# darcamo/pyphysim

Hardware: AMD Instinct MI355X
Metric: Monte Carlo realizations/sec (whole node) + SER abs-error vs ref (higher is better)
Workload: dtype f64

## Files before the change

pyphysim_amd/csrc/bm_f64.hpp:

```cpp
#pragma once
#include <cstdint>

#ifndef MCLE_BM_TABLE
#define MCLE_BM_TABLE static __device__ const
#endif
#ifndef MCLE_BM_FN
#define MCLE_BM_FN __device__ __forceinline__
#endif
#ifndef MCLE_BM_RSQ
#define MCLE_BM_RSQ(a) __builtin_amdgcn_rsq(a)
#endif
#ifndef MCLE_BM_FMA
#define MCLE_BM_FMA(a, b, c) __builtin_fma(a, b, c)
#endif
#ifndef MCLE_BM_RINT
#define MCLE_BM_RINT(a) __builtin_rint(a)
#endif

#ifndef MCLE_BM_ALIGNBIT
#ifdef __HIPCC__
#define MCLE_BM_ALIGNBIT(hi, lo, s) __builtin_amdgcn_alignbit(hi, lo, s)
#else
#define MCLE_BM_ALIGNBIT(hi, lo, s) ((uint32_t)(((((uint64_t)(hi)) << 32) | (uint64_t)(uint32_t)(lo)) >> (s)))
#endif
// ... 115 lines not shown
        st = t[1];
    } else {
        ct = reinterpret_cast<const double*>(entry)[0];
        st = reinterpret_cast<const double*>(entry)[1];
    }
    const double r = ang - *reinterpret_cast<const double*>(reinterpret_cast<const char*>(ttheta) + (off >> 1));
    const double s2 = r * r;
    double p = MCLE_BM_FMA(s2, -1.0 / 5040.0, 1.0 / 120.0);
    p = MCLE_BM_FMA(s2, p, -1.0 / 6.0);
    const double sr = MCLE_BM_FMA(r * s2, p, r);
    double q = MCLE_BM_FMA(s2, -1.0 / 720.0, 1.0 / 24.0);
    q = MCLE_BM_FMA(s2, q, -0.5);
    const double cm = s2 * q;
    c = ct + MCLE_BM_FMA(-st, sr, ct * cm);
    s = st + MCLE_BM_FMA(ct, sr, st * cm);
}

struct BmFetched {
    int d, e;
    uint32_t x1;
    BmPair lg;
    BmPair cs;
    double theta;
};

MCLE_BM_FN BmFetched bm_sample_fetch(uint32_t x0, uint32_t x1, const double* tlogq, const double* ttheta, const double* ttrig) {
    BmFetched t;
    const double ud = (double)x0 + 0.5;
    const uint64_t bits = __builtin_bit_cast(uint64_t, ud);
    const uint32_t hi = (uint32_t)(bits >> 32);
    const uint32_t f = MCLE_BM_ALIGNBIT(hi, (uint32_t)bits, 20);
    t.d = MCLE_BM_SBFE((int)f, 0, 26);
    t.e = (int)(hi + 0x82000u - ((1023u + 32u) << 20)) >> 20;
    const uint32_t offl = (((f >> 1) + (1u << 24)) >> 21) & 0x7F0u;
    t.lg = *reinterpret_cast<const BmPair*>(reinterpret_cast<const char*>(tlogq) + offl);
    t.x1 = x1;
    const uint32_t offt = ((x1 >> 21) + 8u) & 0xFF0u;
    t.cs = *reinterpret_cast<const BmPair*>(reinterpret_cast<const char*>(ttrig) + offt);
    t.theta = *reinterpret_cast<const double*>(reinterpret_cast<const char*>(ttheta) + (offt >> 1));
    return t;
}

MCLE_BM_FN void bm_sample_finish(const BmFetched& t, double sigma, double& re, double& im) {
    const double inv_cq = t.lg[0], lnc = t.lg[1];
    const double r = (double)t.d * inv_cq;
    const double r2 = r * r;
    const double a0 = MCLE_BM_FMA(r, 1.0 / 3.0, -0.5);
    const double a1 = MCLE_BM_FMA(r, 0.2, -0.25);
    const double a2 = MCLE_BM_FMA(r, 1.0 / 7.0, -1.0 / 6.0);
    const double q = MCLE_BM_FMA(r2, MCLE_BM_FMA(r2, a2, a1), a0);
    const double small = MCLE_BM_FMA(r2, q, r);
    const double big = MCLE_BM_FMA((double)t.e, 0x1.62e42fefa39efp-1, lnc);
    const double rad = sigma * bm_sqrt(-(big + small));
    const double ang = (double)t.x1 * 0x1.921fb54442d18p-30;
    const double ct = t.cs[0], st = t.cs[1];
    const double rr = ang - t.theta;
    const double s2 = rr * rr;
    double p = MCLE_BM_FMA(s2, -1.0 / 5040.0, 1.0 / 120.0);
    p = MCLE_BM_FMA(s2, p, -1.0 / 6.0);
    const double sr = MCLE_BM_FMA(rr * s2, p, rr);
    double qq = MCLE_BM_FMA(s2, -1.0 / 720.0, 1.0 / 24.0);
    qq = MCLE_BM_FMA(s2, qq, -0.5);
    const double cm = s2 * qq;
    const double c = ct + MCLE_BM_FMA(-st, sr, ct * cm);
    const double s = st + MCLE_BM_FMA(ct, sr, st * cm);
    re = rad * c;
    im = rad * s;
}

MCLE_BM_FN void bm_sincos_packed(uint32_t x1, double& c, double& s, const double* tpk) {
    const double ang = (double)x1 * 0x1.921fb54442d18p-30;
    const uint32_t k = ((x1 >> 24) + 1u) >> 1;
    const double ct = tpk[4 * k], st = tpk[4 * k + 1];
    const double r = ang - tpk[4 * k + 2];
    const double s2 = r * r;
    double p = MCLE_BM_FMA(s2, -1.0 / 5040.0, 1.0 / 120.0);
    p = MCLE_BM_FMA(s2, p, -1.0 / 6.0);
    const double sr = MCLE_BM_FMA(r * s2, p, r);
    double q = MCLE_BM_FMA(s2, -1.0 / 720.0, 1.0 / 24.0);
    q = MCLE_BM_FMA(s2, q, -0.5);
    const double cm = s2 * q;
    c = ct + MCLE_BM_FMA(-st, sr, ct * cm);
    s = st + MCLE_BM_FMA(ct, sr, st * cm);
}
#ifdef __HIPCC__
constexpr int kBmPackedDoubles = 129 * 4;
__device__ __forceinline__ void bm_trig_packed_to_lds(double* s_pk, int tid, int nthreads) {
    for (int i = tid; i < kBmThetaLen; i += nthreads) {
        s_pk[4 * i] = kBmTrig[2 * i];
        s_pk[4 * i + 1] = kBmTrig[2 * i + 1];
        s_pk[4 * i + 2] = kBmTheta[i];
        s_pk[4 * i + 3] = 0.0;
    }
}
#endif

MCLE_BM_FN void bm_sincos_rad(double x, double& c, double& s) {
    const double C1 = 0x1.45f306dc9c883p-3;
    const double C2 = -0x1.6b01ec5417056p-57;
    const double p = x * C1;
    const double e = MCLE_BM_FMA(x, C1, -p) + x * C2;
    const double kd = MCLE_BM_RINT(p * 4.0);
    const int k = (int)kd;
    const double rt = MCLE_BM_FMA(kd, -0.25, p) + e;
    const double r = rt * 0x1.921fb54442d18p+2;
    const double z = r * r;
// ... 24 lines not shown
```

pyphysim_amd/csrc/philox.hpp:

```cpp
#pragma once
#include "common.hpp"
#include "bm_f64.hpp"

namespace mcle {

enum : uint32_t { STREAM_DATA = 0, STREAM_NOISE = 1, STREAM_CHAN = 2, STREAM_PHASE = 3, STREAM_PILOT = 4 };

struct Words4 {
    uint32_t w[4];
};

__host__ __device__ __forceinline__ Words4 philox4x32_10(uint32_t c0, uint32_t c1, uint32_t c2,
                                                         uint32_t c3, uint32_t k0, uint32_t k1) {
#pragma unroll
    for (int r = 0; r < 10; ++r) {
        const uint64_t p0 = (uint64_t)0xD2511F53u * c0;
        const uint64_t p1 = (uint64_t)0xCD9E8D57u * c2;
#if defined(__HIP_DEVICE_COMPILE__)
        const uint32_t n0 = __builtin_amdgcn_bitop3_b32((uint32_t)(p1 >> 32), c1, k0, 0x96);
        const uint32_t n2 = __builtin_amdgcn_bitop3_b32((uint32_t)(p0 >> 32), c3, k1, 0x96);
#else
        const uint32_t n0 = (uint32_t)(p1 >> 32) ^ c1 ^ k0;
        const uint32_t n2 = (uint32_t)(p0 >> 32) ^ c3 ^ k1;
#endif
// ... 19 lines not shown
          r1((uint32_t)(realization >> 32)) {}
    __host__ __device__ __forceinline__ Words4 block(uint32_t stream, uint32_t blk) const {
        return philox4x32_10(blk, stream, r0, r1, k0, k1);
    }
};

__device__ __forceinline__ float2 cn_from_words(uint32_t x0, uint32_t x1, float sigma) {
    const float u = fmaf((float)x0, 0x1p-32f, 0x1p-33f);
    const float v = (float)x1 * 0x1p-32f;
    const float rad = __builtin_amdgcn_sqrtf((-0.69314718055994531f * sigma * sigma) * __builtin_amdgcn_logf(u));
    float2 z;
    z.x = rad * __builtin_amdgcn_cosf(v);
    z.y = rad * __builtin_amdgcn_sinf(v);
    return z;
}
__device__ __forceinline__ double2 cn_from_words(uint32_t x0, uint32_t x1, double sigma) {
    const double rad = sigma * bm_sqrt(bm_neg_log_q(x0));
    double s, c;
    bm_sincos(x1, c, s);
    double2 z;
    z.x = rad * c;
    z.y = rad * s;
    return z;
}

__device__ __forceinline__ double2 cn_from_words_lds(uint32_t x0, uint32_t x1, double sigma, const double* s_bm) {
    const double rad = sigma * bm_sqrt(bm_neg_log_q(x0, s_bm));
    double s, c;
    bm_sincos(x1, c, s, s_bm + kBmLogLen, s_bm + kBmLogLen + kBmThetaLen);
    double2 z;
    z.x = rad * c;
    z.y = rad * s;
    return z;
}

__device__ __forceinline__ double2 cn_from_words_lds_pairs(uint32_t x0, uint32_t x1, double sigma, const double* s_bm) {
    const double rad = sigma * bm_sqrt(bm_neg_log_q<true>(x0, s_bm));
    double s, c;
    bm_sincos<true>(x1, c, s, s_bm + kBmLogLen + kBmTrigLen, s_bm + kBmLogLen);
    double2 z;
    z.x = rad * c;
    z.y = rad * s;
    return z;
}

__device__ __forceinline__ BmFetched cn_fetch_lds_pairs(uint32_t x0, uint32_t x1, const double* s_bm) {
    return bm_sample_fetch(x0, x1, s_bm, s_bm + kBmLogLen + kBmTrigLen, s_bm + kBmLogLen);
}
__device__ __forceinline__ double2 cn_finish(const BmFetched& t, double sigma) {
    double2 z;
    bm_sample_finish(t, sigma, z.x, z.y);
    return z;
}

template <typename T>
__device__ __forceinline__ cx<T> cn_sample(const Rng& rng, uint32_t stream, uint64_t i, T sigma) {
    const Words4 b = rng.block(stream, (uint32_t)(i >> 1));
    const bool hi = (i & 1) != 0;
    return cn_from_words(hi ? b.w[2] : b.w[0], hi ? b.w[3] : b.w[1], sigma);
}

template <typename T>
__device__ __forceinline__ void cn_pair(const Rng& rng, uint32_t stream, uint32_t blk, T sigma,
                                        cx<T>& z0, cx<T>& z1) {
    const Words4 b = rng.block(stream, blk);
    z0 = cn_from_words(b.w[0], b.w[1], sigma);
    z1 = cn_from_words(b.w[2], b.w[3], sigma);
}

__device__ __forceinline__ void cn_pair_lds(const Rng& rng, uint32_t stream, uint32_t blk, float sigma, float2& z0,
                                            float2& z1, const double*) {
    cn_pair<float>(rng, stream, blk, sigma, z0, z1);
}
__device__ __forceinline__ void cn_pair_lds(const Rng& rng, uint32_t stream, uint32_t blk, double sigma, double2& z0,
                                            double2& z1, const double* s_bm) {
    const Words4 b = rng.block(stream, blk);
    z0 = cn_from_words_lds(b.w[0], b.w[1], sigma, s_bm);
    z1 = cn_from_words_lds(b.w[2], b.w[3], sigma, s_bm);
}

__device__ __forceinline__ float2 cn_one_lds(const Rng& rng, uint32_t stream, uint32_t i, float sigma, const double*) {
    return cn_sample<float>(rng, stream, i, sigma);
}
__device__ __forceinline__ double2 cn_one_lds(const Rng& rng, uint32_t stream, uint32_t i, double sigma, const double* s_bm) {
    const Words4 b = rng.block(stream, i >> 1);
    const bool hi = (i & 1) != 0;
    return cn_from_words_lds(hi ? b.w[2] : b.w[0], hi ? b.w[3] : b.w[1], sigma, s_bm);
}

__device__ __forceinline__ double uniform_at(const Rng& rng, uint32_t stream, uint64_t i) {
    const Words4 b = rng.block(stream, (uint32_t)(i >> 2));
    const uint32_t lo = (i & 1) ? b.w[1] : b.w[0], hi = (i & 1) ? b.w[3] : b.w[2];
    return (double)((i & 2) ? hi : lo) * 0x1p-32;
}

__device__ __forceinline__ uint32_t symbol_at(const Rng& rng, uint64_t n, uint32_t mask) {
    const Words4 b = rng.block(STREAM_DATA, (uint32_t)(n >> 4));
    const uint32_t lo = (n & 4) ? b.w[1] : b.w[0], hi = (n & 4) ? b.w[3] : b.w[2];
    return (((n & 8) ? hi : lo) >> ((n & 3) * 8)) & mask;
}

}
```

pyphysim_amd/csrc/pipeline_mimo_pw.hip:

```cpp
#include "mimo_planar_common.hpp"
#include "walk_f64.hpp"

namespace mcle {

constexpr int kPwPlane = 4 * 272;
__host__ __device__ __forceinline__ int pw_slot(int a, int e) { return a * 272 + e + (e >> 4); }
__host__ __device__ __forceinline__ int pw_mtime(int h, int c) { return (c & 3) * 64 + (c >> 2) * 16 + (h & 3) * 4 + (h >> 2); }
template <int NW> constexpr int pw_lab_stride() { return 16 * NW + 16; }
template <int NW> constexpr size_t pw_static_lds() {
    return (size_t)((kBmLdsDoubles + 1) & ~1) * sizeof(double) + (size_t)64 * pw_lab_stride<NW>() + 2 * (d64_rec<4, 4>() + 1) * sizeof(double2) +
           64 * sizeof(unsigned) + sizeof(WgTotals);
}

__device__ __forceinline__ void pw_row_swap(uint32_t& x, uint32_t& y) {
#if defined(__HIP_DEVICE_COMPILE__)
#if __has_builtin(__builtin_amdgcn_permlane16_swap)
    const auto s = __builtin_amdgcn_permlane16_swap(x, y, false, false);
    x = s[0];
    y = s[1];
#else
    const bool odd = (__lane_id() & 16) != 0;
    const uint32_t give = odd ? x : y, got = (uint32_t)__shfl_xor((int)give, 16);
    if (odd) x = got;
    else y = got;
// ... 56 lines not shown
#pragma unroll
                    for (int q = 0; q < 8; ++q) X[q] = mk<double>((double)(w0 + w1), 1.0);
                } else {
#pragma unroll
                    for (int q = 0; q < 4; ++q) {
                        X[q] = s_txtab[(w0 >> (8 * q)) & 0xFFu];
                        X[q + 4] = s_txtab[(w1 >> (8 * q)) & 0xFFu];
                    }
                }
                double2 A[4];
#pragma unroll
                for (int q = 0; q < 4; ++q) A[q] = (J & 1) ? csub(X[q], X[q + 4]) : cadd(X[q], X[q + 4]);
                const double2 B0 = cadd(A[0], rotJ(A[2])), B1 = cadd(A[1], rotJ(A[3]));
                double2 S;
                if constexpr (J == 0) S = cadd(B0, B1);
                else if constexpr (J == 2) S = mk<double>(B0.x - B1.y, B0.y + B1.x);
                else if constexpr (J == 4) S = csub(B0, B1);
                else if constexpr (J == 6) S = mk<double>(B0.x + B1.y, B0.y - B1.x);
                else {
                    constexpr double c = (J == 1 || J == 7) ? kH : -kH, sn = (J == 1 || J == 3) ? kH : -kH;
                    S = mk<double>(B0.x + (c * B1.x - sn * B1.y), B0.y + (sn * B1.x + c * B1.y));
                }
                if constexpr (J == 0) v[u] = S;
                else if (u == 0) v[u] = S;
                else v[u] = cmulc(S, g_tw[16 * J * u]);
            }
        }
    } else {
        static_assert(NW == 2, "first stage");
#pragma unroll
        for (int i = 0; i < 2; ++i) {
            const uint4 L = lab[i];
            const uint32_t wds[4] = {L.x, L.y, L.z, L.w};
#pragma unroll
            for (int uu = 0; uu < 8; ++uu) {
                const int u = 8 * i + uu;
                const uint32_t w = wds[uu >> 1] >> (16 * (uu & 1));
                double2 X0, X1;
                if constexpr (STUB) {
                    X0 = X1 = mk<double>((double)(w & 0xFFFFu), 1.0);
                } else {
                    X0 = s_txtab[w & 0xFFu];
                    X1 = s_txtab[(w >> 8) & 0xFFu];
                }
                const double2 S = J ? csub(X0, X1) : cadd(X0, X1);
                if constexpr (J == 0) v[u] = S;
                else if (u == 0) v[u] = S;
                else v[u] = cmulc(S, g_tw[16 * J * u]);
            }
        }
    }
}

template <int NW, int DEC, int WPS, bool TD = false, int ABL = 0, bool ROWS = !TD, bool XCH = ROWS && !TD>
__global__ __launch_bounds__(64 * NW, WPS) void k_run_mimo_ofdm_pw(MimoParams pp, ModemParams<double> mp, uint64_t seed, uint64_t first,
                                                                   uint64_t count, const double2* __restrict__ g_tw,
                                                                   const double2* __restrict__ g_recs, mcle_counters* counters,
                                                                   uint32_t* __restrict__ sym_out, uint32_t* __restrict__ bit_out) {
    using T = double;
    constexpr int N = 256 * NW, NT = 4, NR = 4, kRec = d64_rec<NT, NR>(), TB = 64 * NW, UU = 16 / NW;
    constexpr int kLabStride = pw_lab_stride<NW>();
    static_assert(NW == 2 || NW == 4 || NW == 8, "wavefronts per realization");
    static_assert(!(TD && ROWS), "the time-domain form keeps the map wavefront = class");
    static_assert(!XCH || (ROWS && ABL == 0), "the exchange in complex halves belongs to the default form by lane row");
    constexpr bool kAhead = ROWS && ABL == 0;
#ifdef MCLE_PW_LATE_B5
    constexpr bool kLateB5 = XCH && kAhead;
#else
    constexpr bool kLateB5 = false;
#endif
    constexpr int kLogNW = NW == 2 ? 1 : NW == 4 ? 2 : 3;
    extern __shared__ __attribute__((aligned(16))) char pw_smem[];
    constexpr int kBm = (kBmLdsDoubles + 1) & ~1;
    __shared__ __attribute__((aligned(16))) double s_bm[kBm];
    __shared__ __attribute__((aligned(16))) unsigned char s_lab[64 * kLabStride];
    __shared__ __attribute__((aligned(16))) cx<T> s_rec[2 * (kRec + 1)];
    __shared__ unsigned s_part[64];
    __shared__ WgTotals totals;
    static_assert(sizeof(s_bm) + sizeof(s_lab) + sizeof(s_rec) + sizeof(s_part) + sizeof(totals) == pw_static_lds<NW>(), "launcher's LDS sum");
    T* s_R = reinterpret_cast<T*>(pw_smem);
    cx<T>* s_table = reinterpret_cast<cx<T>*>(s_R + NW * kPwPlane);
    cx<T>* s_txtab = s_table + ((mp.M + 1) & ~1);

    const int tid = threadIdx.x, lane = tid & 63;
    const int j = __builtin_amdgcn_readfirstlane(tid >> 6);
    const int pj = j & 1;
    const int cp = pp.cp;
    const int per_sym = N * NT;
    const uint64_t row = (uint64_t)pp.n_ofdm_sym * (N + cp);
    const T sigma = (T)sqrt(pp.noise_var);
    const T tx_scale = (T)(1.0 / sqrt((double)NT) / sqrt((double)(N + cp)));
    const T tab_scale = TD ? tx_scale : tx_scale * (T)N;
    const uint32_t mask = (uint32_t)(mp.M - 1);
    for (int m = tid; m < mp.M; m += TB) {
        const cx<T> c = mp.g_table[m];
        s_table[m] = c;
        s_txtab[m] = cscale(c, tab_scale);
    }
    if constexpr (ROWS) bm_tables_to_lds_pairs(s_bm, tid, TB);
    else bm_tables_to_lds(s_bm, tid, TB);
    if (tid == 0) wg_zero(totals);

    T* s_mine = s_R + j * kPwPlane;
    uint2* s_words_mine = reinterpret_cast<uint2*>(s_mine);
    using Pass = std::conditional_t<kAhead, uint32_t, uint64_t>;
    Pass it = 0;
    uint64_t rl_prev = 0;
    cx<T> rec_next = mk<T>(0, 0);
    if (tid < kRec && blockIdx.x < count) rec_next = g_recs[(uint64_t)blockIdx.x * kRec + tid];
    unsigned step = 0;
    if constexpr (kAhead) {
        step = gridDim.x;
        asm volatile("" : "+s"(step));
    }
    auto grid_step = [&]() -> unsigned {
        if constexpr (kAhead) return step;
        else return gridDim.x;
    };
    __syncthreads();
    for (uint64_t rl = blockIdx.x; rl < count; rl += grid_step(), ++it) {
        const Rng rng(seed, first + rl);
        const int buf = (int)(it & 1);
        if (tid < kRec) {
            s_rec[buf * (kRec + 1) + tid] = rec_next;
            if (rl + grid_step() < count) rec_next = g_recs[(rl + grid_step()) * kRec + tid];
        }
        const cx<T>* s_H = s_rec + buf * (kRec + 1);
        const cx<T>* s_G = s_H + NT * NR;
        unsigned se = 0, be = 0;
        for (int os = 0; os < pp.n_ofdm_sym; ++os) {
            if constexpr (!kLateB5) {
                if (it > 0 || os > 0) __syncthreads();
            }
            if constexpr (ROWS && !(ABL & 128)) __builtin_amdgcn_s_waitcnt(0xC07F);
            {
                const int t = opaque(tid);
                Words4 dw;
                if constexpr (ABL & 32) dw.w[0] = dw.w[1] = dw.w[2] = dw.w[3] = (uint32_t)t * 0x01010101u;
                else dw = rng.block(STREAM_DATA, (uint32_t)(((uint64_t)os * per_sym) >> 4) + (uint32_t)t);
                const int q = (t >> 6) ^ (NW / 2), u = (t & 63) >> 2;
#pragma unroll
                for (int s = 0; s < 4; ++s) {
                    const uint32_t w = dw.w[s] & (mask * 0x01010101u);
                    const int g = 4 * (t & 3) + s;
                    unsigned char* dst = s_lab + g * kLabStride + NW * u + q;
#pragma unroll
                    for (int a = 0; a < 4; ++a) dst[a * 16 * kLabStride] = (unsigned char)(w >> (8 * a));
                }
            }
            if constexpr (!ROWS) {
// ... 88 lines not shown
#pragma unroll
                for (int u = 0; u < 16; ++u) s_mine[wbase + 17 * u] = v[u].x;
                walk_wave_order();
#pragma unroll
                for (int c = 0; c < 16; ++c) xr[c] = s_mine[rbase + c];
                walk_wave_order();
#pragma unroll
                for (int u = 0; u < 16; ++u) s_mine[wbase + 17 * u] = v[u].y;
                walk_wave_order();
#pragma unroll
                for (int c = 0; c < 16; ++c) v[c] = mk<T>(xr[c], s_mine[rbase + c]);
            }
            if constexpr (TD && !(ABL & 64)) {
                R16Tw64<T> none;
                r16_pass<T, true, false, 0, false, true, true, false, true>(nullptr, nullptr, 0, none, nullptr, 0, v, v);
            }
            if constexpr (!TD && !ROWS) {
#pragma unroll
                for (int c = 0; c < 16; ++c) {
                    if constexpr (ABL & 128) v[c] = mk<T>((T)nw[c].x, sigma);
                    else v[c] = cn_words(nw[c].x, nw[c].y, sigma, s_bm);
                }
            }
            if constexpr (ROWS) {
                const int ln = opaque(lane);
                const int rho = ln >> 4, h = ln & 15;
                const int f = 4 * j + rho, ant = f >> kLogNW, cls = f & (NW - 1);
                const uint64_t i00 = (uint64_t)ant * row + (uint64_t)os * (N + cp) + cp + (cls & ~1) + 32 * NW * (rho & 1) + NW * (uint64_t)pw_mtime(h, 0);
                const uint32_t b0 = (uint32_t)(i00 >> 1);
                if constexpr (ABL & 128) {
#pragma unroll
                    for (int cc = 0; cc < 8; ++cc) {
                        Words4 b;
                        b.w[0] = b.w[1] = b.w[2] = b.w[3] = b0 + cc;
                        pw_row_swap(b.w[0], b.w[2]);
                        pw_row_swap(b.w[1], b.w[3]);
                        v[cc] = mk<T>((T)b.w[0], sigma);
                        v[8 + cc] = mk<T>((T)b.w[2], sigma);
                    }
                } else {
                    BmFetched ft[8][2];
                    auto fetch = [&](int cc) {
                        Words4 b = rng.block(STREAM_NOISE, b0 + (uint32_t)(NW / 2) * (uint32_t)pw_mtime(0, cc));
                        pw_row_swap(b.w[0], b.w[2]);
                        pw_row_swap(b.w[1], b.w[3]);
                        ft[cc][0] = cn_fetch_lds_pairs(b.w[0], b.w[1], s_bm);
                        ft[cc][1] = cn_fetch_lds_pairs(b.w[2], b.w[3], s_bm);
                    };
                    fetch(0);
#pragma unroll
                    for (int cc = 0; cc < 8; ++cc) {
                        if (cc + 1 < 8) fetch(cc + 1);
                        __builtin_amdgcn_sched_barrier(0);
                        v[cc] = cn_finish(ft[cc][0], sigma);
                        v[8 + cc] = cn_finish(ft[cc][1], sigma);
                        __builtin_amdgcn_sched_barrier(0);
                    }
                }
            }
            if constexpr (TD) {
                const int ln = opaque(lane);
                const cx<T> hA = s_H[(ln & 3) * NT + (ln >> 4)];
                const T hre = hA.x, him = hA.y, nhim = -hA.y;
#pragma unroll
                for (int c = 0; c < 16; ++c) {
                    cx<T> z;
                    if constexpr (ABL & 128) z = mk<T>((T)nw[c].x, sigma);
                    else z = cn_words(nw[c].x, nw[c].y, sigma, s_bm);
                    if constexpr (ABL & 256) {
                        v[c] = cadd(v[c], z);
                    } else {
                        T yr = __builtin_amdgcn_mfma_f64_4x4x4f64(hre, v[c].x, z.x, 0, 0, 0);
                        T yi = __builtin_amdgcn_mfma_f64_4x4x4f64(him, v[c].x, z.y, 0, 0, 0);
                        yr = __builtin_amdgcn_mfma_f64_4x4x4f64(nhim, v[c].y, yr, 0, 0, 0);
                        yi = __builtin_amdgcn_mfma_f64_4x4x4f64(hre, v[c].y, yi, 0, 0, 0);
                        v[c] = mk<T>(yr, yi);
                    }
                }
            }
            R16Tw64<T> tw1;
            if constexpr (kAhead) {
                const int g = opaque(lane) & 15;
#pragma unroll
                for (int m = 1; m <= 3; ++m) {
                    tw1.a1[m - 1] = g_tw[NW * g * m];
                    tw1.a2[m - 1] = g_tw[4 * NW * g * m];
                }
                __builtin_amdgcn_sched_barrier(0);
            }
            if constexpr (!(ABL & 512)) {
                R16Tw64<T> none;
                r16_pass<T, false, true, 0, false, true, true, false, true>(nullptr, nullptr, 0, none, nullptr, 0, v, v);
            }
            {
                const int ln = opaque(lane);
                const int a = ln >> 4, g = ln & 15;
                const int wbase = pw_slot(a, g), rbase = pw_slot(a, 16 * g);
                T xr[16];
                if constexpr (kLateB5) {
#pragma unroll
                    for (int c = 0; c < 16; ++c) asm volatile("" : "+v"(v[c].x), "+v"(v[c].y));
                    if (it > 0 || os > 0) __syncthreads();
                }
#pragma unroll
                for (int c = 0; c < 16; ++c) s_mine[rbase + c] = v[c].x;
                walk_wave_order();
#pragma unroll
                for (int u = 0; u < 16; ++u) xr[u] = s_mine[wbase + 17 * u];
// ... 111 lines not shown
                    else return tw_at(m, uu);
                };
#pragma unroll
                for (int uu = 0; uu < UU; ++uu) {
                    if constexpr (kAhead) {
                        if (uu + 1 < UU) {
#pragma unroll
                            for (int m = 1; m < NW; ++m) twb[(uu + 1) & 1][m - 1] = tw_at(m, uu + 1);
                        }
                        __builtin_amdgcn_sched_barrier(0);
                    }
                    if constexpr (NW == 4) {
                        const cx<T> w1 = tw_of(1, uu), w2 = tw_of(2, uu), w3 = tw_of(3, uu);
                        const cx<T> u0 = ex(0, uu);
                        const cx<T> u1 = cmul(ex(1, uu), w1);
                        const cx<T> u2 = cmul(ex(2, uu), w2);
                        const cx<T> u3 = cmul(ex(3, uu), w3);
                        CxOps<T>::template bfly4<false>(u0, u1, u2, u3, v[4 * uu], v[4 * uu + 1], v[4 * uu + 2], v[4 * uu + 3]);
                    } else if constexpr (NW == 8) {
                        cx<T> x[8];
                        x[0] = ex(0, uu);
#pragma unroll
                        for (int jj = 1; jj < 8; ++jj) x[jj] = cmul(ex(jj, uu), tw_of(jj, uu));
                        cx<T> E[4], O[4];
                        CxOps<T>::template bfly4<false>(x[0], x[2], x[4], x[6], E[0], E[1], E[2], E[3]);
                        CxOps<T>::template bfly4<false>(x[1], x[3], x[5], x[7], O[0], O[1], O[2], O[3]);
                        constexpr T kH = (T)0.70710678118654752440;
                        const cx<T> t0 = O[0];
                        const cx<T> t1 = mk<T>(kH * (O[1].x + O[1].y), kH * (O[1].y - O[1].x));
                        const cx<T> t2 = mk<T>(O[2].y, -O[2].x);
                        const cx<T> t3 = mk<T>(kH * (O[3].y - O[3].x), -kH * (O[3].x + O[3].y));
                        v[8 * uu + 0] = cadd(E[0], t0); v[8 * uu + 4] = csub(E[0], t0);
                        v[8 * uu + 1] = cadd(E[1], t1); v[8 * uu + 5] = csub(E[1], t1);
                        v[8 * uu + 2] = cadd(E[2], t2); v[8 * uu + 6] = csub(E[2], t2);
                        v[8 * uu + 3] = cadd(E[3], t3); v[8 * uu + 7] = csub(E[3], t3);
                    } else {
                        const cx<T> u0 = ex(0, uu);
                        const cx<T> u1 = cmul(ex(1, uu), tw_of(1, uu));
                        v[2 * uu] = cadd(u0, u1);
                        v[2 * uu + 1] = csub(u0, u1);
                    }
                }
            }
            {
                const int ln = opaque(lane);
                uint4 L;
                if constexpr (kAhead) L = lab_ahead;
                else L = *reinterpret_cast<const uint4*>(s_lab + ln * kLabStride + 16 * j);
                const uint32_t wds[4] = {L.x, L.y, L.z, L.w};
                if constexpr (!TD && !(ABL & 256)) {
                    cx<T> hA;
                    if constexpr (kAhead) hA = hA_ahead;
                    else hA = s_H[(ln & 3) * NT + (ln >> 4)];
                    const T hre = hA.x, him = hA.y, nhim = -hA.y;
#pragma unroll
                    for (int i = 0; i < 4; ++i) {
                        cx<T> X[4];
#pragma unroll
                        for (int jj = 0; jj < 4; ++jj) {
                            const uint32_t lb = (wds[i] >> (8 * jj)) & 0xFFu;
                            if constexpr (ABL & 32) X[jj] = mk<T>((T)lb, 1.0);
                            else X[jj] = s_txtab[lb];
                        }
                        T yr[4], yi[4];
#pragma unroll
                        for (int jj = 0; jj < 4; ++jj) {
                            yr[jj] = __builtin_amdgcn_mfma_f64_4x4x4f64(hre, X[jj].x, v[4 * i + jj].x, 0, 0, 0);
                            yi[jj] = __builtin_amdgcn_mfma_f64_4x4x4f64(him, X[jj].x, v[4 * i + jj].y, 0, 0, 0);
                        }
#pragma unroll
                        for (int jj = 0; jj < 4; ++jj) {
                            yr[jj] = __builtin_amdgcn_mfma_f64_4x4x4f64(nhim, X[jj].y, yr[jj], 0, 0, 0);
                            yi[jj] = __builtin_amdgcn_mfma_f64_4x4x4f64(hre, X[jj].y, yi[jj], 0, 0, 0);
                            v[4 * i + jj] = mk<T>(yr[jj], yi[jj]);
                        }
                    }
                }
                if constexpr (!(ABL & 1024)) {
                cx<T> gA;
                if constexpr (kAhead) gA = gA_ahead;
                else gA = s_G[(ln & 3) * NR + (ln >> 4)];
                const T gre = gA.x, gim = gA.y, ngim = -gA.y;
#pragma unroll
                for (int i = 0; i < 4; ++i) {
                    cx<T> e[4];
#pragma unroll
                    for (int jj = 0; jj < 4; ++jj) {
                        const int u = 4 * i + jj;
                        T xr = __builtin_amdgcn_mfma_f64_4x4x4f64(gre, v[u].x, 0.0, 0, 0, 0);
                        T xi = __builtin_amdgcn_mfma_f64_4x4x4f64(gim, v[u].x, 0.0, 0, 0, 0);
                        xr = __builtin_amdgcn_mfma_f64_4x4x4f64(ngim, v[u].y, xr, 0, 0, 0);
                        xi = __builtin_amdgcn_mfma_f64_4x4x4f64(gre, v[u].y, xi, 0, 0, 0);
                        e[jj] = mk<T>(xr, xi);
                    }
                    if constexpr (DEC == WDEC_SLICER || DEC == WDEC_QAM_CERT) {
                        walk_qam_count4<DEC == WDEC_QAM_CERT>(mp, s_table, e, wds[i], se, be);
                    } else {
                        int tx[4];
#pragma unroll
                        for (int jj = 0; jj < 4; ++jj) tx[jj] = (int)((wds[i] >> (8 * jj)) & 0xFFu);
                        walk_decide<DEC, 4>(mp, s_table, nullptr, e, tx, se, be);
                    }
                }
                } else {
                    T keep = er[0][0] + ei[NW - 1][UU - 1];
                    if constexpr (!TD) {
#pragma unroll
                        for (int u = 0; u < 16; ++u) keep += v[u].x + v[u].y;
                    }
                    se += (unsigned)(keep == 0.5) + (wds[0] == 0x12345u);
                }
            }
        }
        if constexpr (kAhead) {
            se = walk_wave_total(se);
            be = walk_wave_total(be);
        } else {
            se = wave_sum_u32(se);
            be = wave_sum_u32(be);
        }
        if (lane == 0) {
            s_part[buf * 32 + 2 * j] = se;
            s_part[buf * 32 + 2 * j + 1] = be;
        }
        rl_prev = rl;
    }
    __syncthreads();
    if (tid == 0) {
        if (it > 0) {
            const int buf = (int)((it - 1) & 1);
            const unsigned* qq = s_part + buf * 32;
            unsigned ts = 0, tb = 0;
#pragma unroll
            for (int i = 0; i < NW; ++i) {
                ts += qq[2 * i];
                tb += qq[2 * i + 1];
            }
            if constexpr (kAhead) rl_prev = blockIdx.x + (uint64_t)(it - 1) * step;
            wg_account(totals, ts, tb, s_rec[buf * (kRec + 1) + 2 * NT * NR].x != 0.0, rl_prev, sym_out, bit_out);
        }
        wg_flush(totals, counters, (unsigned long long)per_sym * pp.n_ofdm_sym, (unsigned long long)per_sym * pp.n_ofdm_sym * mp.bits);
    }
}

template <int NW, int WPS, bool TD, int ABL, bool ROWS, bool XCH>
static int launch_mimo_ofdm_pw(mcle_ctx* ctx, const C4Plan& plan, const mcle_mimo_ofdm_cfg* cfg, uint64_t seed, uint64_t first,
                               uint64_t count, mcle_counters* d_counters, uint32_t* d_sym, uint32_t* d_bit) {
    using T = double;
    constexpr int N = 256 * NW, NT = 4, NR = 4;
    int rc;
    void* tw = nullptr;
    if ((rc = ctx->get_twiddles(N, MCLE_F64, &tw))) return rc;
    MimoParams pp{cfg->cp_size, cfg->num_used, cfg->n_ofdm_sym, cfg->mmse, cfg->noise_var};
    ModemParams<T> mp = pipe_modem<T>(ctx, cfg->demod_method);
    const int dec = walk_dec_kind(ctx, mp);
    mp.grid.G = 0;
    const size_t tab_len = ((size_t)mp.M + 1) & ~(size_t)1;
    const size_t dyn = (size_t)NW * kPwPlane * sizeof(T) + 2 * tab_len * sizeof(cx<T>);
    const size_t lds = dyn + pw_static_lds<NW>();
    MCLE_REQUIRE(lds + 512 <= (size_t)160 * 1024, "part-wave MIMO-OFDM kernel: %zu B of LDS do not fit", lds);
    auto kern = k_run_mimo_ofdm_pw<NW, WDEC_SLICER, WPS, TD, ABL, ROWS, XCH>;
    switch (dec) {
        case WDEC_QAM_CERT: kern = k_run_mimo_ofdm_pw<NW, WDEC_QAM_CERT, WPS, TD, ABL, ROWS, XCH>; break;
        case WDEC_QUAD_CERT: kern = k_run_mimo_ofdm_pw<NW, WDEC_QUAD_CERT, WPS, TD, ABL, ROWS, XCH>; break;
        case WDEC_AXIS4_CERT: kern = k_run_mimo_ofdm_pw<NW, WDEC_AXIS4_CERT, WPS, TD, ABL, ROWS, XCH>; break;
        default: break;
    }
    MCLE_HIP(hipFuncSetAttribute((const void*)kern, hipFuncAttributeMaxDynamicSharedMemorySize, (int)dyn));
    int per_cu = (int)((size_t)160 * 1024 / (lds + 512));
    if (per_cu < 1) per_cu = 1;
    const int by_waves = WPS * 4 / NW;
    if (per_cu > by_waves) per_cu = by_waves;
    const uint64_t resident = (uint64_t)ctx->n_cu * per_cu;
    static_assert(XCH ? ROWS && ABL == 0 : true, "the exchange in complex halves: default form by lane row only");
    set_c4_kernel(ctx, plan);
    const uint64_t kSlice = 1ull << 20;
    return launch_sliced_planar<T, N, NT, NR>(ctx, pp, seed, first, count, kSlice, d_sym, d_bit,
                                              [&](void* recs, uint64_t at, uint64_t n, uint32_t* sym, uint32_t* bit) {
        const unsigned grid = (unsigned)oversubscribed_grid(ctx, resident, n, 8, NW == 4 ? 32 : 16);
        hipLaunchKernelGGL(kern, dim3(grid), dim3(64 * NW), dyn, ctx->stream, pp, mp, seed, at, n, (const cx<T>*)tw, (const cx<T>*)recs,
                           d_counters, sym, bit);
    });
}

int launch_mimo_ofdm_pw(mcle_ctx* ctx, const C4Plan& p, const mcle_mimo_ofdm_cfg* cfg, uint64_t seed, uint64_t first, uint64_t count,
                        mcle_counters* d_counters, uint32_t* d_sym, uint32_t* d_bit) {
#define MCLE_PW(NW_, WPS_, TD_, ABL_, ROWS_, XCH_)                                                                              \
    if (p.n == 256 * NW_ && p.wps == WPS_ && p.td == TD_ && p.abl == ABL_ && p.rows == ROWS_ && p.halves == XCH_)               \
        return launch_mimo_ofdm_pw<NW_, WPS_, TD_, ABL_, ROWS_, XCH_>(ctx, p, cfg, seed, first, count, d_counters, d_sym, d_bit);
#define MCLE_PW_SIZE(NW_, WPS_)                                                                                                 \
    MCLE_PW(NW_, WPS_, false, 0, false, false) MCLE_PW(NW_, WPS_, false, 0, true, true) MCLE_PW(NW_, WPS_, false, 0, true, false) \
    MCLE_PW(NW_, WPS_, true, 0, false, false)
    MCLE_PW_SIZE(2, 3) MCLE_PW(2, 2, false, 0, true, false)
    MCLE_PW_SIZE(4, 3) MCLE_PW(4, 2, false, 0, true, true)
    MCLE_PW_SIZE(8, 2)
#ifdef MCLE_EXPERIMENTS
#define MCLE_PW_ABL(V_)                                                                                                         \
    MCLE_PW(2, 3, true, V_, false, false) MCLE_PW(2, 3, false, V_, true, false) MCLE_PW(4, 3, true, V_, false, false)           \
    MCLE_PW(4, 3, false, V_, true, false)
    MCLE_PW_ABL(32) MCLE_PW_ABL(64) MCLE_PW_ABL(128) MCLE_PW_ABL(256) MCLE_PW_ABL(512) MCLE_PW_ABL(1024) MCLE_PW_ABL(2016)
#undef MCLE_PW_ABL
#endif
#undef MCLE_PW_SIZE
#undef MCLE_PW
    MCLE_REQUIRE(false, "internal: no part-wave MIMO-OFDM kernel <%d> w%d time %d rows %d halves %d ablation %d", p.n / 256, p.wps, (int)p.td,
                 (int)p.rows, (int)p.halves, p.abl);
}

}
```

pyphysim_amd/csrc/walk_f64.hpp:

```cpp
#pragma once
#include <cmath>
#include "modem.hpp"
#include "philox.hpp"
#include "totals.hpp"
#include "pipe_common.hpp"
#include "qam_pack.hpp"
#include "wave_draws.hpp"

namespace mcle {

template <typename T> inline int walk_dec_kind(const mcle_ctx* ctx, ModemParams<T>& mp) {
    if (mp.method == MCLE_DEMOD_QAM_SLICER) return WDEC_SLICER;
    if (mp.cert == 1) return WDEC_QAM_CERT;
    if (mp.cert == 2) return WDEC_QUAD_CERT;
    if (mp.method == MCLE_DEMOD_MINDIST && ctx->axis_ok && !ctx->opt[MCLE_OPT_DEMOD_NOCERT]) {
        mp.quad_lut = ctx->axis_lut;
        mp.quad_lo = (T)(ctx->axis_a * (sizeof(T) == 8 ? 0x1p-30 : 0x1p-15));
        mp.quad_hi = (T)(ctx->axis_a * (sizeof(T) == 8 ? 0x1p+8 : 8.0));
        return WDEC_AXIS4_CERT;
    }
    return WDEC_GENERIC;
}

__device__ __forceinline__ void walk_wave_order() {
    __builtin_amdgcn_fence(__ATOMIC_RELEASE, "wavefront");
    __builtin_amdgcn_wave_barrier();
    __builtin_amdgcn_fence(__ATOMIC_ACQUIRE, "wavefront");
}

__device__ __forceinline__ uint32_t walk_wave_total(uint32_t v) {
    v += (uint32_t)__builtin_amdgcn_update_dpp(0, (int)v, 0x111, 0xF, 0xF, true);
    v += (uint32_t)__builtin_amdgcn_update_dpp(0, (int)v, 0x112, 0xF, 0xF, true);
    v += (uint32_t)__builtin_amdgcn_update_dpp(0, (int)v, 0x114, 0xF, 0xF, true);
    v += (uint32_t)__builtin_amdgcn_update_dpp(0, (int)v, 0x118, 0xF, 0xF, true);
    v += (uint32_t)__builtin_amdgcn_update_dpp(0, (int)v, 0x142, 0xA, 0xF, true);
    v += (uint32_t)__builtin_amdgcn_update_dpp(0, (int)v, 0x143, 0xC, 0xF, true);
    return (uint32_t)__builtin_amdgcn_readlane((int)v, 63);
}

template <typename T> __device__ __forceinline__ int walk_sweep(const cx<T>* __restrict__ s_table, int M, cx<T> r) {
    T best = dist2(r, s_table[0]);
    int idx = 0;
#pragma unroll 1
    for (int m = 1; m < M; ++m) {
        const T d = dist2(r, s_table[m]);
        if (d < best) {
            best = d;
            idx = m;
        }
    }
    return idx;
}

__device__ __forceinline__ int walk_qam_slicer(float2 r, float scale, int L, int half_bits) {
// ... 37 lines not shown
            kj = (int)floor(fmin(fmax(tj, (T)0), lm1));
            ki = (int)floor(fmin(fmax(ti, (T)0), lm1));
        }
        lv |= (((uint32_t)ki << hb) | (uint32_t)kj) << (8 * i);
    }
    if constexpr (CERT) {
        if (!all) {
            const uint32_t g1 = ((fm >> 1) | ((fm >> 1) << hb)) & 0xFFu;
#pragma unroll
            for (int i = 0; i < 4; ++i)
                if (!sure[i]) {
                    const uint32_t lab = (uint32_t)walk_sweep<T>(s_table, mp.M, e[i]);
                    const uint32_t lev = lab ^ ((lab >> 1) & g1);
                    lv = (lv & ~(0xFFu << (8 * i))) | (lev << (8 * i));
                }
        }
    }
    return lv;
}

constexpr int kWalkFixShift = 24;
constexpr uint32_t kWalkFixDelta = 2u;
__device__ __forceinline__ int walk_fix_q(double x, int lo, int hi) {
    int q = 0;
#if defined(__HIP_DEVICE_COMPILE__)
    asm("v_cvt_i32_f64 %0, %1\n\tv_med3_i32 %0, %0, %2, %3" : "=&v"(q) : "v"(x), "v"(lo), "s"(hi));
#endif
    return q;
}
__device__ __forceinline__ bool walk_qam_fixed4(const ModemParams<double>& mp, const double2 (&e)[4], uint32_t& lv) {
    constexpr int S = kWalkFixShift;
    constexpr uint32_t kOff = (0u - kWalkFixDelta) << 8, kBound = ((1u << S) - 1u - 2u * kWalkFixDelta) << 8;
    const double hs = mp.qam_scale * 0.5, hl = (double)(mp.qam_L - 1) * 0.5;
    const double c1 = hs * (double)(1 << S), c0 = (hl + 0.5) * (double)(1 << S);
    const int lo = 1 << (S - 1), hi = ((mp.qam_L - 1) << S) + (1 << (S - 1));
    int qj[4], qi[4];
    uint32_t worst = 0u;
#pragma unroll
    for (int i = 0; i < 4; ++i) {
        qj[i] = walk_fix_q(__builtin_fma(e[i].x, c1, c0), lo, hi);
        qi[i] = walk_fix_q(__builtin_fma(e[i].y, -c1, c0), lo, hi);
        const uint32_t fj = ((uint32_t)qj[i] << 8) + kOff, fi = ((uint32_t)qi[i] << 8) + kOff;
        worst = max(max(worst, fj), fi);
    }
    const uint32_t j01 = __builtin_amdgcn_perm((uint32_t)qj[1], (uint32_t)qj[0], 0x0c0c0703u);
    const uint32_t j23 = __builtin_amdgcn_perm((uint32_t)qj[3], (uint32_t)qj[2], 0x0c0c0703u);
    const uint32_t i01 = __builtin_amdgcn_perm((uint32_t)qi[1], (uint32_t)qi[0], 0x0c0c0703u);
    const uint32_t i23 = __builtin_amdgcn_perm((uint32_t)qi[3], (uint32_t)qi[2], 0x0c0c0703u);
    const uint32_t wj = __builtin_amdgcn_perm(j23, j01, 0x05040100u), wi = __builtin_amdgcn_perm(i23, i01, 0x05040100u);
    lv = (wi << mp.half_bits) | wj;
    return worst <= kBound;
}

template <typename T, bool CERT>
__device__ __forceinline__ void walk_qam_count4(const ModemParams<T>& mp, const cx<T>* __restrict__ s_table, const cx<T> (&e)[4],
                                                uint32_t sent, unsigned& se, unsigned& be) {
    static_assert(sizeof(T) == 8 || CERT, "complex64 slices in the packed form (qam_levels4)");
    const int hb = mp.half_bits;
    const uint32_t fm = (1u << hb) - 1u;
    QamPack qp;
    qp.hb = hb;
    qp.m1 = (((fm >> 1) | ((fm >> 1) << hb)) & 0xFFu) * 0x01010101u;
    qp.m2 = (((fm >> 2) | ((fm >> 2) << hb)) & 0xFFu) * 0x01010101u;
    uint32_t lv;
    if constexpr (CERT && sizeof(T) == 8) {
        if (__builtin_expect(!walk_qam_fixed4(mp, e, lv), 0)) lv = walk_qam_levels4<T, CERT>(mp, s_table, e);
    } else {
        lv = walk_qam_levels4<T, CERT>(mp, s_table, e);
    }
    qam_count4(lv ^ labels_to_levels(sent, qp), qp, se, be);
}
template <bool CERT>
__device__ __forceinline__ void walk_qam_count4(const ModemParams<double>& mp, const double2* __restrict__ s_table, const double2 (&e)[4],
                                                uint32_t sent, unsigned& se, unsigned& be) {
    walk_qam_count4<double, CERT>(mp, s_table, e, sent, se, be);
}

template <typename T, int DEC, int N>
__device__ __forceinline__ void walk_decide(const ModemParams<T>& mp, const cx<T>* __restrict__ s_table,
                                            const unsigned long long* __restrict__ s_grid, const cx<T> (&e)[N],
                                            const int (&tx)[N], unsigned& se, unsigned& be) {
    if constexpr (DEC == WDEC_SLICER && sizeof(T) == 4) {
        const QamPack qp = qam_pack(mp);
#pragma unroll
        for (int g0 = 0; g0 < N; g0 += 4) {
            f4q er = {0.f, 0.f, 0.f, 0.f}, ei = {0.f, 0.f, 0.f, 0.f};
            uint32_t sent = 0u;
#pragma unroll
            for (int i = 0; i < 4; ++i)
                if (g0 + i < N) {
                    er[i] = e[g0 + i].x;
                    ei[i] = e[g0 + i].y;
                    sent |= (uint32_t)tx[g0 + i] << (8 * i);
                }
            const uint32_t live = N - g0 >= 4 ? 0xFFFFFFFFu : ((1u << (8 * ((N - g0) & 3))) - 1u);
            qam_count4((qam_levels4(er, ei, qp) ^ labels_to_levels(sent, qp)) & live, qp, se, be);
        }
        return;
    }
    if constexpr ((sizeof(T) == 8 ? (DEC == WDEC_SLICER || DEC == WDEC_QAM_CERT) : DEC == WDEC_QAM_CERT) && N % 4 == 0) {
#pragma unroll
        for (int g0 = 0; g0 < N; g0 += 4) {
            const cx<T> e4[4] = {e[g0], e[g0 + 1], e[g0 + 2], e[g0 + 3]};
            const uint32_t sent = (uint32_t)tx[g0] | ((uint32_t)tx[g0 + 1] << 8) | ((uint32_t)tx[g0 + 2] << 16) | ((uint32_t)tx[g0 + 3] << 24);
            walk_qam_count4<T, DEC == WDEC_QAM_CERT>(mp, s_table, e4, sent, se, be);
        }
        return;
    }
    int dec[N];
    if constexpr (DEC == WDEC_SLICER) {
#pragma unroll
        for (int j = 0; j < N; ++j) dec[j] = walk_qam_slicer(e[j], mp.qam_scale, mp.qam_L, mp.half_bits);
    } else if constexpr (DEC == WDEC_QAM_CERT || DEC == WDEC_QUAD_CERT || DEC == WDEC_AXIS4_CERT) {
        bool sure[N], all = true;
#pragma unroll
        for (int j = 0; j < N; ++j) {
            if constexpr (DEC == WDEC_QAM_CERT) dec[j] = demod_qam_cert<T>(e[j], mp.qam_scale, mp.qam_L, mp.half_bits, sure[j]);
            else if constexpr (DEC == WDEC_QUAD_CERT) dec[j] = demod_quad_cert<T>(e[j], mp.quad_lut, mp.quad_lo, mp.quad_hi, sure[j]);
            else dec[j] = demod_axis4_cert<T>(e[j], mp.quad_lut, mp.quad_lo, mp.quad_hi, sure[j]);
            all = all && sure[j];
        }
        if (!all) {
// ... 295 lines not shown
```

Baseline: 50.45 million.

## Fold noise scale and QAM fixed-point affine map into MFMA operands

Adds a FIX variant of the MIMO OFDM pairwise kernel. It draws unit-variance noise and folds sigma into the transmit table, and uses the MFMA negate modifiers instead of explicit negation. It also folds the slicer's affine scale and offset (c1, c0) into the equalizer MFMA, so the accumulator directly holds fixed-point slicer coordinates. This removes per-sample multiplies and adds ahead of the fixed-point QAM decision. The cost is a wave-wide max reduction, a host-computed gain cap, an s_nop settle, and a fallback path that recomputes the symbols when the certificate fails.

```diff
diff --git a/pyphysim_amd/csrc/bm_f64.hpp b/pyphysim_amd/csrc/bm_f64.hpp
--- a/pyphysim_amd/csrc/bm_f64.hpp
+++ b/pyphysim_amd/csrc/bm_f64.hpp
@@ -191,6 +191,33 @@
     const double small = MCLE_BM_FMA(r2, q, r);
     const double big = MCLE_BM_FMA((double)t.e, 0x1.62e42fefa39efp-1, lnc);
     const double rad = sigma * bm_sqrt(-(big + small));
+    const double ang = (double)t.x1 * 0x1.921fb54442d18p-30;
+    const double ct = t.cs[0], st = t.cs[1];
+    const double rr = ang - t.theta;
+    const double s2 = rr * rr;
+    double p = MCLE_BM_FMA(s2, -1.0 / 5040.0, 1.0 / 120.0);
+    p = MCLE_BM_FMA(s2, p, -1.0 / 6.0);
+    const double sr = MCLE_BM_FMA(rr * s2, p, rr);
+    double qq = MCLE_BM_FMA(s2, -1.0 / 720.0, 1.0 / 24.0);
+    qq = MCLE_BM_FMA(s2, qq, -0.5);
+    const double cm = s2 * qq;
+    const double c = ct + MCLE_BM_FMA(-st, sr, ct * cm);
+    const double s = st + MCLE_BM_FMA(ct, sr, st * cm);
+    re = rad * c;
+    im = rad * s;
+}
+
+MCLE_BM_FN void bm_sample_finish_unit(const BmFetched& t, double& re, double& im) {
+    const double inv_cq = t.lg[0], lnc = t.lg[1];
+    const double r = (double)t.d * inv_cq;
+    const double r2 = r * r;
+    const double a0 = MCLE_BM_FMA(r, 1.0 / 3.0, -0.5);
+    const double a1 = MCLE_BM_FMA(r, 0.2, -0.25);
+    const double a2 = MCLE_BM_FMA(r, 1.0 / 7.0, -1.0 / 6.0);
+    const double q = MCLE_BM_FMA(r2, MCLE_BM_FMA(r2, a2, a1), a0);
+    const double small = MCLE_BM_FMA(r2, q, r);
+    const double big = MCLE_BM_FMA((double)t.e, 0x1.62e42fefa39efp-1, lnc);
+    const double rad = bm_sqrt(-(big + small));
     const double ang = (double)t.x1 * 0x1.921fb54442d18p-30;
     const double ct = t.cs[0], st = t.cs[1];
     const double rr = ang - t.theta;
diff --git a/pyphysim_amd/csrc/philox.hpp b/pyphysim_amd/csrc/philox.hpp
--- a/pyphysim_amd/csrc/philox.hpp
+++ b/pyphysim_amd/csrc/philox.hpp
@@ -95,6 +95,11 @@
     bm_sample_finish(t, sigma, z.x, z.y);
     return z;
 }
+__device__ __forceinline__ double2 cn_finish_unit(const BmFetched& t) {
+    double2 z;
+    bm_sample_finish_unit(t, z.x, z.y);
+    return z;
+}
 
 template <typename T>
 __device__ __forceinline__ cx<T> cn_sample(const Rng& rng, uint32_t stream, uint64_t i, T sigma) {
diff --git a/pyphysim_amd/csrc/pipeline_mimo_pw.hip b/pyphysim_amd/csrc/pipeline_mimo_pw.hip
--- a/pyphysim_amd/csrc/pipeline_mimo_pw.hip
+++ b/pyphysim_amd/csrc/pipeline_mimo_pw.hip
@@ -132,7 +132,7 @@
     }
 }
 
-template <int NW, int DEC, int WPS, bool TD = false, int ABL = 0, bool ROWS = !TD, bool XCH = ROWS && !TD>
+template <int NW, int DEC, int WPS, bool TD = false, int ABL = 0, bool ROWS = !TD, bool XCH = ROWS && !TD, bool FIX = false>
 __global__ __launch_bounds__(64 * NW, WPS) void k_run_mimo_ofdm_pw(MimoParams pp, ModemParams<double> mp, uint64_t seed, uint64_t first,
                                                                    uint64_t count, const double2* __restrict__ g_tw,
                                                                    const double2* __restrict__ g_recs, mcle_counters* counters,
@@ -144,6 +144,7 @@
     static_assert(!(TD && ROWS), "the time-domain form keeps the map wavefront = class");
     static_assert(!XCH || (ROWS && ABL == 0), "the exchange in complex halves belongs to the default form by lane row");
     constexpr bool kAhead = ROWS && ABL == 0;
+    static_assert(!FIX || (kAhead && DEC == WDEC_QAM_CERT), "the scales on the matrix-core operands: default form by lane row, QAM certificate");
 #ifdef MCLE_PW_LATE_B5
     constexpr bool kLateB5 = XCH && kAhead;
 #else
@@ -175,7 +176,8 @@
     for (int m = tid; m < mp.M; m += TB) {
         const cx<T> c = mp.g_table[m];
         s_table[m] = c;
-        s_txtab[m] = cscale(c, tab_scale);
+        if constexpr (FIX) s_txtab[m] = cscale(c, tab_scale / sigma);
+        else s_txtab[m] = cscale(c, tab_scale);
     }
     if constexpr (ROWS) bm_tables_to_lds_pairs(s_bm, tid, TB);
     else bm_tables_to_lds(s_bm, tid, TB);
@@ -370,8 +372,13 @@
                     for (int cc = 0; cc < 8; ++cc) {
                         if (cc + 1 < 8) fetch(cc + 1);
                         __builtin_amdgcn_sched_barrier(0);
-                        v[cc] = cn_finish(ft[cc][0], sigma);
-                        v[8 + cc] = cn_finish(ft[cc][1], sigma);
+                        if constexpr (FIX) {
+                            v[cc] = cn_finish_unit(ft[cc][0]);
+                            v[8 + cc] = cn_finish_unit(ft[cc][1]);
+                        } else {
+                            v[cc] = cn_finish(ft[cc][0], sigma);
+                            v[8 + cc] = cn_finish(ft[cc][1], sigma);
+                        }
                         __builtin_amdgcn_sched_barrier(0);
                     }
                 }
@@ -589,7 +596,9 @@
                     cx<T> hA;
                     if constexpr (kAhead) hA = hA_ahead;
                     else hA = s_H[(ln & 3) * NT + (ln >> 4)];
-                    const T hre = hA.x, him = hA.y, nhim = -hA.y;
+                    const T hre = hA.x, him = hA.y;
+                    [[maybe_unused]] T nhim = 0;
+                    if constexpr (!FIX) nhim = -hA.y;
 #pragma unroll
                     for (int i = 0; i < 4; ++i) {
                         cx<T> X[4];
@@ -607,7 +616,8 @@
                         }
 #pragma unroll
                         for (int jj = 0; jj < 4; ++jj) {
-                            yr[jj] = __builtin_amdgcn_mfma_f64_4x4x4f64(nhim, X[jj].y, yr[jj], 0, 0, 0);
+                            if constexpr (FIX) yr[jj] = __builtin_amdgcn_mfma_f64_4x4x4f64(him, X[jj].y, yr[jj], 0, 0, 1);
+                            else yr[jj] = __builtin_amdgcn_mfma_f64_4x4x4f64(nhim, X[jj].y, yr[jj], 0, 0, 0);
                             yi[jj] = __builtin_amdgcn_mfma_f64_4x4x4f64(hre, X[jj].y, yi[jj], 0, 0, 0);
                             v[4 * i + jj] = mk<T>(yr[jj], yi[jj]);
                         }
@@ -617,6 +627,45 @@
                 cx<T> gA;
                 if constexpr (kAhead) gA = gA_ahead;
                 else gA = s_G[(ln & 3) * NR + (ln >> 4)];
+                if constexpr (FIX) {
+                    const T sc1 = sigma * walk_fix_c1(mp.qam_scale), c0 = walk_fix_c0(mp.qam_L);
+                    const T g2re = gA.x * sc1, g2im = gA.y * sc1;
+                    const uint32_t hw = max((uint32_t)__double2hiint(g2re) & 0x7FFFFFFFu, (uint32_t)__double2hiint(g2im) & 0x7FFFFFFFu);
+                    const bool over = walk_wave_max(hw) >= mp.quad_lut;
+#pragma unroll
+                    for (int i = 0; i < 4; ++i) {
+                        T dj[4], di[4];
+#pragma unroll
+                        for (int jj = 0; jj < 4; ++jj) {
+                            const int u = 4 * i + jj;
+                            T xr = __builtin_amdgcn_mfma_f64_4x4x4f64(g2re, v[u].x, c0, 0, 0, 0);
+                            T xi = __builtin_amdgcn_mfma_f64_4x4x4f64(g2im, v[u].x, c0, 0, 0, 1);
+                            xr = __builtin_amdgcn_mfma_f64_4x4x4f64(g2im, v[u].y, xr, 0, 0, 1);
+                            xi = __builtin_amdgcn_mfma_f64_4x4x4f64(g2re, v[u].y, xi, 0, 0, 1);
+                            dj[jj] = xr;
+                            di[jj] = xi;
+                        }
+                        walk_mfma_settle8(dj, di);
+                        uint32_t lv;
+                        const bool ok = walk_qam_fixed4_delivered(mp, dj, di, lv) && !over;
+                        if (__builtin_expect(__builtin_amdgcn_ballot_w64(!ok) != 0, 0)) {
+                            const cx<T> gB = s_G[(ln & 3) * NR + (ln >> 4)];
+                            const T sre = gB.x * sigma, sim = gB.y * sigma;
+                            cx<T> e[4];
+#pragma unroll
+                            for (int jj = 0; jj < 4; ++jj) {
+                                const int u = 4 * i + jj;
+                                T xr = __builtin_amdgcn_mfma_f64_4x4x4f64(sre, v[u].x, 0.0, 0, 0, 0);
+                                T xi = __builtin_amdgcn_mfma_f64_4x4x4f64(sim, v[u].x, 0.0, 0, 0, 0);
+                                xr = __builtin_amdgcn_mfma_f64_4x4x4f64(sim, v[u].y, xr, 0, 0, 1);
+                                xi = __builtin_amdgcn_mfma_f64_4x4x4f64(sre, v[u].y, xi, 0, 0, 0);
+                                e[jj] = mk<T>(xr, xi);
+                            }
+                            lv = walk_qam_levels4<T, true>(mp, s_table, e);
+                        }
+                        walk_qam_count_levels4(mp, lv, wds[i], se, be);
+                    }
+                } else {
                 const T gre = gA.x, gim = gA.y, ngim = -gA.y;
 #pragma unroll
                 for (int i = 0; i < 4; ++i) {
@@ -638,6 +687,7 @@
                         for (int jj = 0; jj < 4; ++jj) tx[jj] = (int)((wds[i] >> (8 * jj)) & 0xFFu);
                         walk_decide<DEC, 4>(mp, s_table, nullptr, e, tx, se, be);
                     }
+                }
                 }
                 } else {
                     T keep = er[0][0] + ei[NW - 1][UU - 1];
@@ -703,6 +753,16 @@
         case WDEC_AXIS4_CERT: kern = k_run_mimo_ofdm_pw<NW, WDEC_AXIS4_CERT, WPS, TD, ABL, ROWS, XCH>; break;
         default: break;
     }
+#ifndef MCLE_PW_SCALES
+#define MCLE_PW_SCALES 1
+#endif
+    if constexpr (MCLE_PW_SCALES && ROWS && !TD && ABL == 0 && (XCH || NW == 2)) {
+        if (dec == WDEC_QAM_CERT && cfg->noise_var > 0.0 && plan.asked != 'x') {
+            kern = k_run_mimo_ofdm_pw<NW, WDEC_QAM_CERT, WPS, TD, ABL, ROWS, XCH, true>;
+            const double tab_scale = 1.0 / std::sqrt((double)NT) / std::sqrt((double)(N + cfg->cp_size)) * (double)N;
+            mp.quad_lut = pw_fixed_gcap_hi((double)mp.qam_scale, mp.qam_L, N, tab_scale, std::sqrt(cfg->noise_var));
+        }
+    }
     MCLE_HIP(hipFuncSetAttribute((const void*)kern, hipFuncAttributeMaxDynamicSharedMemorySize, (int)dyn));
     int per_cu = (int)((size_t)160 * 1024 / (lds + 512));
     if (per_cu < 1) per_cu = 1;
diff --git a/pyphysim_amd/csrc/walk_f64.hpp b/pyphysim_amd/csrc/walk_f64.hpp
--- a/pyphysim_amd/csrc/walk_f64.hpp
+++ b/pyphysim_amd/csrc/walk_f64.hpp
@@ -1,5 +1,6 @@
 #pragma once
 #include <cmath>
+#include <cstring>
 #include "modem.hpp"
 #include "philox.hpp"
 #include "totals.hpp"
@@ -143,6 +144,59 @@
     return worst <= kBound;
 }
 
+__host__ __device__ __forceinline__ double walk_fix_c1(double qam_scale) { return qam_scale * 0.5 * (double)(1 << kWalkFixShift); }
+__host__ __device__ __forceinline__ double walk_fix_c0(int qam_L) { return ((double)(qam_L - 1) * 0.5 + 0.5) * (double)(1 << kWalkFixShift); }
+
+inline uint32_t pw_fixed_gcap_hi(double qam_scale, int qam_L, int n, double tab_scale, double sigma) {
+    const double R = std::sqrt(33.0 * 0.69314718055994530942);
+    const double xmax = 1.4142135623730951 * (double)(qam_L - 1) / qam_scale;
+    const double ymax = (4.0 * R * xmax * tab_scale / sigma + (double)n * R) * (1.0 + 0x1p-20);
+    const double gcap = (0x1p40 - walk_fix_c0(qam_L)) / (8.0 * ymax);
+    uint64_t bits;
+    std::memcpy(&bits, &gcap, sizeof bits);
+    return (uint32_t)(bits >> 32);
+}
+
+__device__ __forceinline__ void walk_mfma_settle8(double (&dj)[4], double (&di)[4]) {
+#if defined(__HIP_DEVICE_COMPILE__)
+    asm volatile("s_nop 7"
+                 : "+v"(dj[0]), "+v"(dj[1]), "+v"(dj[2]), "+v"(dj[3]), "+v"(di[0]), "+v"(di[1]), "+v"(di[2]), "+v"(di[3]));
+#endif
+}
+
+__device__ __forceinline__ bool walk_qam_fixed4_delivered(const ModemParams<double>& mp, const double (&dj)[4], const double (&di)[4],
+                                                          uint32_t& lv) {
+    constexpr int S = kWalkFixShift;
+    constexpr uint32_t kOff = (0u - kWalkFixDelta) << 8, kBound = ((1u << S) - 1u - 2u * kWalkFixDelta) << 8;
+    const int lo = 1 << (S - 1), hi = ((mp.qam_L - 1) << S) + (1 << (S - 1));
+    int qj[4], qi[4];
+    uint32_t worst = 0u;
+#pragma unroll
+    for (int i = 0; i < 4; ++i) {
+        qj[i] = walk_fix_q(dj[i], lo, hi);
+        qi[i] = walk_fix_q(di[i], lo, hi);
+        const uint32_t fj = ((uint32_t)qj[i] << 8) + kOff, fi = ((uint32_t)qi[i] << 8) + kOff;
+        worst = max(max(worst, fj), fi);
+    }
+    const uint32_t j01 = __builtin_amdgcn_perm((uint32_t)qj[1], (uint32_t)qj[0], 0x0c0c0703u);
+    const uint32_t j23 = __builtin_amdgcn_perm((uint32_t)qj[3], (uint32_t)qj[2], 0x0c0c0703u);
+    const uint32_t i01 = __builtin_amdgcn_perm((uint32_t)qi[1], (uint32_t)qi[0], 0x0c0c0703u);
+    const uint32_t i23 = __builtin_amdgcn_perm((uint32_t)qi[3], (uint32_t)qi[2], 0x0c0c0703u);
+    const uint32_t wj = __builtin_amdgcn_perm(j23, j01, 0x05040100u), wi = __builtin_amdgcn_perm(i23, i01, 0x05040100u);
+    lv = (wi << mp.half_bits) | wj;
+    return worst <= kBound;
+}
+
+__device__ __forceinline__ uint32_t walk_wave_max(uint32_t v) {
+    v = max(v, (uint32_t)__builtin_amdgcn_update_dpp(0, (int)v, 0x111, 0xF, 0xF, true));
+    v = max(v, (uint32_t)__builtin_amdgcn_update_dpp(0, (int)v, 0x112, 0xF, 0xF, true));
+    v = max(v, (uint32_t)__builtin_amdgcn_update_dpp(0, (int)v, 0x114, 0xF, 0xF, true));
+    v = max(v, (uint32_t)__builtin_amdgcn_update_dpp(0, (int)v, 0x118, 0xF, 0xF, true));
+    v = max(v, (uint32_t)__builtin_amdgcn_update_dpp(0, (int)v, 0x142, 0xA, 0xF, true));
+    v = max(v, (uint32_t)__builtin_amdgcn_update_dpp(0, (int)v, 0x143, 0xC, 0xF, true));
+    return (uint32_t)__builtin_amdgcn_readlane((int)v, 63);
+}
+
 template <typename T, bool CERT>
 __device__ __forceinline__ void walk_qam_count4(const ModemParams<T>& mp, const cx<T>* __restrict__ s_table, const cx<T> (&e)[4],
                                                 uint32_t sent, unsigned& se, unsigned& be) {
@@ -159,6 +213,15 @@
     } else {
         lv = walk_qam_levels4<T, CERT>(mp, s_table, e);
     }
+    qam_count4(lv ^ labels_to_levels(sent, qp), qp, se, be);
+}
+__device__ __forceinline__ void walk_qam_count_levels4(const ModemParams<double>& mp, uint32_t lv, uint32_t sent, unsigned& se, unsigned& be) {
+    const int hb = mp.half_bits;
+    const uint32_t fm = (1u << hb) - 1u;
+    QamPack qp;
+    qp.hb = hb;
+    qp.m1 = (((fm >> 1) | ((fm >> 1) << hb)) & 0xFFu) * 0x01010101u;
+    qp.m2 = (((fm >> 2) | ((fm >> 2) << hb)) & 0xFFu) * 0x01010101u;
     qam_count4(lv ^ labels_to_levels(sent, qp), qp, se, be);
 }
 template <bool CERT>
```

Result: no change. 50.85 million (median of 6 runs) (+0.8%).
